# THUDM/GRAND-plus

Measured on AMD Instinct MI355X. Metric: propagation-matrix rows/sec (whole node), higher is better.
Workload: dtype f64

## Files before the change

### grand_plus_amd/csrc/gfpush.hip

```cpp
#include "gfpush_kernels.hpp"
#include "gfpush_sketch.hpp"
#include "gfpush_plan.hpp"
#include "grandplus.h"

#include <dlfcn.h>
#include <sys/prctl.h>
#include <rccl/rccl.h>

#include <algorithm>
#include <atomic>
#include <cmath>
#include <cstdarg>
#include <cstdio>
#include <cstdlib>
#include <cstring>
#include <new>
#include <string>
#include <chrono>
#include <thread>
#include <type_traits>
#include <vector>

using namespace gp;
using namespace gp::planning;
// ... 498 lines not shown
        Held held = g->ws.held();
        bool realloc = false; int need = 0; std::string err;
        Status st;
        while ((st = plan_general(kConsts, in, g->opt, shape, occ, sk, p, g->est, held, &realloc, &need, err)) == kNeedOccupancy) {
            int rc = resident_blocks(general_kernel(p.block_threads), p.block_threads, p.lds_bytes + g->opt.lds_pad, &occ.general[need]);
            if (rc) return rc;
        }
        if (st) return plan_status(st, err);
        if (!realloc) return GP_OK;
        int rc = allocate_workspace(g, held);
        if (rc == GP_ERR_NOMEM && sk.use && !shape.insists_on_sketch()) {
            sk.use = false; g_last_error.clear();
            continue;
        }
        return rc;
    }
}

KParams call_params(const gp_graph* g, const CallArgs& a, const GeneralPlan& gk, u64* counters)
{
    KParams kp;
    std::memset(&kp, 0, sizeof kp);
    kp.indptr = g->d_indptr; kp.indices = g->d_indices; kp.n_nodes = (int)g->n_nodes; kp.nnz = (int)g->nnz;
    kp.deg_shift = g->deg_shift; kp.node_mask = g->node_mask; kp.deg_sat = g->deg_sat;
    kp.seeds = a.d_seeds; kp.n_seeds = a.n_seeds;
    kp.coef = g->d_coef; kp.n_coef = a.n_coef; kp.rmax = a.rmax; kp.K = a.K;
    kp.out_row = a.d_row; kp.out_col = a.d_col; kp.out_val = a.d_val; kp.out_filled = a.d_filled;
    kp.counters = counters;
    kp.lds_slots = gk.lds_slots;
    kp.force_global = g->opt.force_global;
    kp.prune = prune_allowed(g->opt, a.coef, a.n_coef) ? 1 : 0;
    kp.diag_flags = g->opt.diag_flags;
    kp.rows_distinct = g->rows_distinct && g->opt.seedrow ? 1u : 0u;
    kp.solo = (g->opt.solo_levels ? 1u : 0u) | (g->opt.sk_seed_merge ? 2u : 0u);
    kp.direct = direct_tables(g->opt, g->n_nodes, gk) ? 1 : 0;
    return kp;
}

struct GeneralPass { const u32* rows; int n_rows; int queue; u32* overflow; int n_overflow; int overflow_queue; const u32* order; };

int launch_general(const gp_graph* g, KParams& kp, const GeneralPlan& gk, bool gk_acsr, const GeneralPass& pass, hipStream_t s)
{
    const Workspace& w = g->ws;
    const bool two_tier = w.big.n_wg > 0;
    use_csr(kp, g, gk_acsr, true);
    use_slabs(kp, w.est);
    kp.row_map = pass.rows ? pass.rows : pass.order; kp.n_rows_dev = pass.rows ? kp.counters + pass.n_rows : nullptr; kp.queue_counter = pass.queue;
    kp.retry_list = two_tier ? pass.overflow : nullptr; kp.retry_counter = pass.n_overflow;
    const Kernel k = pass.rows ? retry_kernel(gk.block_threads) : general_kernel(gk.block_threads);
    int rc = launch_kernel(k, gk.block_threads, kp, gk.n_wg, gk.lds_bytes + g->opt.lds_pad, s);
    if (rc || !two_tier) return rc;
    use_slabs(kp, w.big);
    kp.row_map = pass.overflow; kp.n_rows_dev = kp.counters + pass.n_overflow; kp.queue_counter = pass.overflow_queue;
    kp.retry_list = nullptr;
    return launch_kernel(retry_kernel(gk.block_threads), gk.block_threads, kp, w.big.n_wg, gk.lds_bytes + g->opt.lds_pad, s);
}

int enqueue_row_order(gp_graph* g, const CallArgs& a, bool acsr, hipStream_t s)
{
    const Workspace& w = g->ws;
    HIP_TRY(hipMemsetAsync(w.order_hist, 0, sizeof(uint32_t) * 64, s));
    const int shift = acsr ? g->a_shift : g->deg_shift;
    const u32 sat = acsr ? g->a_sat : g->deg_sat;
    const unsigned cost_wgs = (unsigned)std::min<int64_t>((a.n_seeds + 15) / 16, 4096), order_wgs = (unsigned)std::min<int64_t>((a.n_seeds + 255) / 256, 1024);
    hipLaunchKernelGGL(row_cost_kernel, dim3(cost_wgs), dim3(256), 0, s, a.d_seeds, (long long)a.n_seeds, (int)g->n_nodes, g->d_indptr,
                       acsr ? g->d_acsr : g->d_indices, acsr ? g->d_node_pos : (const u32*)nullptr, shift, sat, a.rmax, w.cost_cls, w.order_hist);
    hipLaunchKernelGGL(row_order_kernel, dim3(order_wgs), dim3(256), 0, s, w.cost_cls, (long long)a.n_seeds, w.order_hist, w.order_hist + 32, w.order);
// ... 363 lines not shown
            if (!value && g->shared_devices) return fail(GP_ERR_INVALID_ARG, "parts of this handle share a device: RCCL takes one rank per device, the gather stays on the host");
            g->gather_host = value ? 1 : 0; return GP_OK;
        }
        if (k == "min_rows_per_gpu") {
            if (value < 1) return fail(GP_ERR_INVALID_ARG, "min_rows_per_gpu must be >= 1");
            g->min_rows_per_gpu = value; return GP_OK;
        }
        for (gp_graph* q : g->part) if (q) { int rc = gp_set_option(q, key, value); if (rc) return rc; }
        return GP_OK;
    }
    if (k == "block_threads") {
        if (value != 256 && value != 512 && value != 768 && value != 1024) return fail(GP_ERR_INVALID_ARG, "block_threads must be 256, 512, 768 or 1024");
        g->opt.block_threads = (int)value;
    } else if (k == "lds_bytes") {
        if (value < 40 * 1024 || value > 160 * 1024) return fail(GP_ERR_INVALID_ARG, "lds_bytes must be in [40960, 163840]");
        g->opt.lds_bytes = (int)(value & ~15ll);
    } else if (k == "lds_pad") {
        if (value < 0 || value > 120 * 1024) return fail(GP_ERR_INVALID_ARG, "lds_pad must be in [0, 122880]");
        g->opt.lds_pad = (int)(value & ~15ll);
    } else if (k == "kernel") {
        if (value < 0 || value > 2) return fail(GP_ERR_INVALID_ARG, "kernel must be 0 (automatic), 1 (general) or 2 (sketch)");
        g->opt.kernel = (int)value;
    } else if (k == "sk_block_threads") {
        if (value != 0 && value != 512 && value != 768 && value != 1024) return fail(GP_ERR_INVALID_ARG, "sk_block_threads must be 0, 512, 768 or 1024");
        g->opt.sk_block = (int)value;
    } else if (k == "sk_lg_mu" || k == "sk_lg_mr") {
        if (value != 0 && (value < 8 || value > 14)) return fail(GP_ERR_INVALID_ARG, "%s must be 0 or in [8, 14]", key);
        (k == "sk_lg_mu" ? g->opt.sk_lg_mu : g->opt.sk_lg_mr) = (int)value;
    } else if (k == "sk_direct_max") {
        if (value < 0 || value > (1 << 20)) return fail(GP_ERR_INVALID_ARG, "sk_direct_max must be in [0, 2^20]");
        g->opt.sk_direct_max = (int)value;
    } else if (k == "sk_seed_merge") {
        g->opt.sk_seed_merge = value ? 1 : 0;
    } else if (k == "row_order") {
        g->opt.row_order = value ? 1 : 0;
    } else if (k == "gk_acsr") {
        g->opt.gk_acsr = value ? 1 : 0;
    } else if (k == "sk_target") {
        if (value < 0 || value > 4096) return fail(GP_ERR_INVALID_ARG, "sk_target must be in [0, 4096]");
        g->opt.sk_target = (int)value;
    } else if (k == "measure_choice") {
        g->opt.measure_choice = value ? 1 : 0;
        if (!value) g->choices.clear();
    } else if (k == "verify_merge") {
        g->opt.verify_merge = value ? 1 : 0;
    } else if (k == "pretouch") {
        g->opt.pretouch = value ? 1 : 0;
    } else if (k == "max_workgroups") {
        if (value < 0 || value > 65535) return fail(GP_ERR_INVALID_ARG, "max_workgroups must be in [0, 65535]");
        g->opt.max_workgroups = (int)value;
    } else if (k == "workspace_mb") {
        if (value < 1) return fail(GP_ERR_INVALID_ARG, "workspace_mb must be >= 1");
        g->opt.workspace_mb = value;
    } else if (k == "est_level_edges") {
        if (value < 0) return fail(GP_ERR_INVALID_ARG, "est_level_edges must be >= 0");
        g->opt.est_level_edges = value;
    } else if (k == "force_global") {
        g->opt.force_global = value ? 1 : 0;
    } else if (k == "exact_stats") {
        g->opt.exact_stats = value ? 1 : 0;
    } else if (k == "direct_tables") {
        g->opt.direct_tables = value ? 1 : 0;
    } else if (k == "solo_levels") {
        g->opt.solo_levels = value ? 1 : 0;
    } else if (k == "seedrow") {
        g->opt.seedrow = value ? 1 : 0;
// ... 210 lines not shown
    *out = nullptr;
    const int ndev = gp_device_count();
    if (ndev <= 0) return fail(GP_ERR_NO_DEVICE, "no HIP device is visible (this library has no CPU path)");
    if (n_gpus < 0 || n_gpus > ndev) return fail(GP_ERR_NO_DEVICE, "n_gpus = %d but %d device(s) are visible", n_gpus, ndev);
    if (n_gpus == 0) n_gpus = ndev;
    std::vector<int> devs(n_gpus);
    for (int d = 0; d < n_gpus; ++d) devs[d] = d;
    return gp_graph_create_multi_on(indptr, n_nodes, indices, nnz, devs.data(), n_gpus, out);
}

}

namespace {

int replicate_part(gp_graph* g, int d) {
    gp_graph* src = g->part[0];
    HIP_TRY(hipSetDevice(src->device));
    int rc = ensure_packed(src, src->stream);
    if (rc) return rc;
    HIP_TRY(hipStreamSynchronize(src->stream));
    const int dev = g->devices[d];
    HIP_TRY(hipSetDevice(dev));
    hipDeviceProp_t prop;
    HIP_TRY(hipGetDeviceProperties(&prop, dev));
    gp_graph* q = new (std::nothrow) gp_graph();
    if (!q) return fail(GP_ERR_NOMEM, "host allocation failed");
    struct Guard { gp_graph* q; ~Guard() { if (q) gp_graph_destroy(q); } } guard{q};
    q->device = dev; q->n_nodes = src->n_nodes; q->nnz = src->nnz; q->num_cus = prop.multiProcessorCount;
    q->deg_shift = src->deg_shift; q->node_mask = src->node_mask; q->deg_sat = src->deg_sat;
    q->packed = true; q->opt.max_degree_bits = src->opt.max_degree_bits; q->rows_distinct = src->rows_distinct;
    q->opt.block_threads = src->opt.block_threads; q->opt.lds_bytes = src->opt.lds_bytes; q->opt.max_workgroups = src->opt.max_workgroups;
    q->opt.workspace_mb = src->opt.workspace_mb; q->opt.force_global = src->opt.force_global; q->opt.exact_stats = src->opt.exact_stats;
    q->opt.direct_tables = src->opt.direct_tables; q->opt.est_level_edges = src->opt.est_level_edges; q->opt.seedrow = src->opt.seedrow; q->opt.solo_levels = src->opt.solo_levels;
    q->opt.kernel = src->opt.kernel; q->opt.row_order = src->opt.row_order; q->opt.gk_acsr = src->opt.gk_acsr; q->opt.sk_seed_merge = src->opt.sk_seed_merge; q->opt.sk_block = src->opt.sk_block; q->opt.sk_lg_mu = src->opt.sk_lg_mu; q->opt.sk_lg_mr = src->opt.sk_lg_mr; q->opt.sk_target = src->opt.sk_target; q->opt.lds_pad = src->opt.lds_pad; q->opt.sk_direct_max = src->opt.sk_direct_max;
    const size_t b_ptr = sizeof(int) * (size_t)(q->n_nodes + 1), b_idx = sizeof(int) * (size_t)(q->nnz + 1);
    HIP_TRY(hipMalloc(&q->d_indptr, b_ptr));
    HIP_TRY(hipMalloc(&q->d_indices, b_idx));
    if (dev == src->device) {
        HIP_TRY(hipMemcpy(q->d_indptr, src->d_indptr, b_ptr, hipMemcpyDeviceToDevice));
        HIP_TRY(hipMemcpy(q->d_indices, src->d_indices, b_idx, hipMemcpyDeviceToDevice));
    } else {
        HIP_TRY(hipMemcpyPeer(q->d_indptr, dev, src->d_indptr, src->device, b_ptr));
        HIP_TRY(hipMemcpyPeer(q->d_indices, dev, src->d_indices, src->device, b_idx));
    }
    HIP_TRY(hipMalloc(&q->d_counters, sizeof(u64) * kNumCounters));
    HIP_TRY(hipHostMalloc(&q->h_counters, sizeof(u64) * kNumCounters));
    HIP_TRY(hipEventCreate(&q->ev0));
    HIP_TRY(hipEventCreate(&q->ev1));
    HIP_TRY(hipStreamCreateWithFlags(&q->stream, hipStreamNonBlocking));
    guard.q = nullptr;
    g->part[d] = q;
    return GP_OK;
}

int gfpush_multi(gp_graph* g, const int32_t* seeds, int64_t n_seeds, const double* coef, int n_coef, double rmax, int K,
                 int32_t* row_idx, int32_t* col_idx, double* value)
{
    const MultiPlan plan = plan_multi(n_seeds, K, g->n_parts, g->min_rows_per_gpu, g->force_collective != 0, g->gather_host != 0);
    const int G = plan.G, Gc = plan.Gc;
    if (plan.single) {
        int rc = gp_gfpush(g->part[0], seeds, n_seeds, coef, n_coef, rmax, K, row_idx, col_idx, value);
        gp_stats st; const int rc2 = gp_get_stats(g->part[0], &st);
        g->m_last = st; g->m_has_stats = true;
        return rc ? rc : rc2;
    }
    const bool collective = !g->gather_host;
    for (int d = 1; d < Gc; ++d)
// ... 104 lines not shown
```

### grand_plus_amd/csrc/gfpush_plan.hpp

```cpp
#pragma once

#include <algorithm>
#include <atomic>
#include <cmath>
#include <cstddef>
#include <cstdint>
#include <cstdio>
#include <cstring>
#include <string>

namespace gp {
namespace planning {

typedef unsigned long long cap_t;

enum Status { kOk = 0, kInvalidArg, kNoMem, kNeedOccupancy };

struct KernelConsts {
    int ctl_bytes = 0, three_lds = 0, min_cap = 0, topk_bins = 0, bucket_cap = 0, unit_shift = 0;
    int sk_max_pushers = 0, sk_max_coef = 0, sk_tie = 0;
};

struct Options {
    int block_threads = 0; int lds_bytes = 0; int max_workgroups = 0;
    int verify_merge = 0;
    int lds_pad = 0; int pretouch = 0;
    int64_t workspace_mb = 65536; int force_global = 0; int exact_stats = 0; int diag_flags = 0; int direct_tables = 1; int seedrow = 1; int solo_levels = 1;
    int kernel = 0;
    int sk_block = 0, sk_lg_mu = 0, sk_lg_mr = 0, sk_target = 0, sk_direct_max = 0;
    int row_order = 1;
    int sk_seed_merge = 1; int gk_acsr = 1;
    int64_t est_level_edges = 0;
    int measure_choice = 1;
    int max_degree_bits = 31;
};

struct Estimate {
    int kind = 0; int last_kind = 1;
    bool sk_auto_off = false; double sk_off_rmax = 0.0; int sk_off_n_coef = 0;
    bool last_sk_soft = false;
    double edges = 0.0, log = 0.0;
    double rmax = -1.0; int n_coef = 0;
    bool recipe_changed = false;
    double cur_edges = 0.0, cur_log = 0.0;
    int64_t last_call_rows = 0; bool grown_for_call = true;
};


struct SlabCaps {
    int n_wg = 0;
    cap_t push_cap = 0, resg_cap = 0, log_cap = 0, cand_cap = 0, bucket_cap = 0, bt_cap = 0;
    cap_t arch_cap = 0;
    size_t log_bytes() const { return arch_cap ? 6 * (size_t)log_cap + 8 * (size_t)arch_cap : 12 * (size_t)log_cap; }
    size_t per_wg() const { return 16 * (size_t)(2 * push_cap + resg_cap + cand_cap + bucket_cap) + log_bytes() + 8 * (size_t)bt_cap + 64; }
    bool covers(const SlabCaps& o) const {
        if (o.n_wg == 0) return true;
        return n_wg >= o.n_wg && push_cap >= o.push_cap && resg_cap >= o.resg_cap && log_cap >= o.log_cap &&
               cand_cap >= o.cand_cap && bucket_cap >= o.bucket_cap && bt_cap >= o.bt_cap && arch_cap >= o.arch_cap && (arch_cap != 0) == (o.arch_cap != 0);
    }
    void widen(const SlabCaps& o) {
        if (o.n_wg == 0 || (n_wg != 0 && (arch_cap != 0) != (o.arch_cap != 0))) return;
        n_wg = std::max(n_wg, o.n_wg); push_cap = std::max(push_cap, o.push_cap); resg_cap = std::max(resg_cap, o.resg_cap);
        log_cap = std::max(log_cap, o.log_cap); cand_cap = std::max(cand_cap, o.cand_cap); bucket_cap = std::max(bucket_cap, o.bucket_cap);
// ... 422 lines not shown
```

### grand_plus_amd/csrc/gfpush_sketch.hpp

```cpp
#pragma once

#include "gfpush_kernels.hpp"

#ifndef GP_DIAG

namespace gp {

#ifndef GP_SK_SWEEP_DEPTH
#define GP_SK_SWEEP_DEPTH 2
#endif
constexpr int kSkMaxCoef = 40;
constexpr u32 kSkTie     = 256;

struct CtlS {
    long long row;
    LevelCtr lc[2];
    u32 ovf;
    u32 fail;
    u32 n_sel, n_tie;
    u32 tk_bin, tk_above, tk_count, tk_total;
    u32 tk_t, tk_wide, tk_dig;
    u64 kth_bits;
    u32 bcnt[64];
    u64 st[8], st_row[8];
    double coef[kSkMaxCoef + 1];
    u32 cand_q[kSkMaxCoef];
    int seed_key; u32 tot_pu, tot_log;
    double lv_dang; u32 lv_has_dang;
    u32 max_e, max_log;
    u32 k_log_cap, k_pu_cap, k_direct_max, k_solo_ok, k_cx, k_pad; double k_rscale;
#ifdef GP_SK_TIMING
    u64 tacc[16]; u64 tlast;
    u64 tacc2[14]; u64 tlast2;
    u64 t_enter, t_row, row_sum, row_max;
    u64 row_hist[32];
#endif
};
#ifdef GP_SK_TIMING
#define SKT_BEGIN(ctl) do { if (threadIdx.x == 0) (ctl)->tlast = wall_clock64(); } while (0)
#define SKT(ctl, i) do { if (threadIdx.x == 0) { const u64 n_ = wall_clock64(); (ctl)->tacc[i] += n_ - (ctl)->tlast; (ctl)->tlast = n_; } } while (0)
#define SKT_COUNT(ctl, i, n) do { if (threadIdx.x == 0) (ctl)->tacc[i] += (n); } while (0)
#define SKT2_BEGIN(ctl) do { if (threadIdx.x == 0) (ctl)->tlast2 = wall_clock64(); } while (0)
#define SKT2(ctl, i) do { if (threadIdx.x == 0) { const u64 n_ = wall_clock64(); (ctl)->tacc2[i] += n_ - (ctl)->tlast2; (ctl)->tlast2 = n_; } } while (0)
#else
#define SKT_BEGIN(ctl) do { } while (0)
#define SKT(ctl, i) do { } while (0)
#define SKT_COUNT(ctl, i, n) do { } while (0)
#define SKT2_BEGIN(ctl) do { } while (0)
#define SKT2(ctl, i) do { } while (0)
#endif
static_assert(sizeof(CtlS) <= (size_t)kCtlStruct, "the control block must fit its LDS reservation");
enum StatS { zPush = 0, zEdges, zDeg, zFilled, zLevels, zFailed, zCand, zSweep2, zNumStats };
__device__ __forceinline__ void zstat(CtlS* ctl, int which, u64 n) {
    __hip_atomic_fetch_add(&ctl->st_row[which], n, __ATOMIC_RELAXED, __HIP_MEMORY_SCOPE_WORKGROUP);
}

struct SkView {
    CtlS* ctl; u32* R; u32* U; double* xvals; int* xkeys; u32 MU, MR, CX, shU, shR;
    PushEntry* push2; u32* bt2; int* log_key; unsigned short* log_pu; double* arch;
    u32 lds_u;
    u32* bt_l; u32 bt_l_cap;
};
template <int BLOCK>
__device__ __forceinline__ SkView sk_view(KP p, u32 lds0) {
    SkView w;
    w.MU = 1u << p.sk_lg_mu; w.MR = 1u << p.sk_lg_mr; w.CX = p.sk_cx;
    w.shU = 32u - p.sk_lg_mu; w.shR = 32u - p.sk_lg_mr;
    w.ctl = lds_at<CtlS>(lds0);
    w.R = lds_at<u32>(lds0 + (u32)kCtlBytes);
    w.lds_u = lds0 + (u32)kCtlBytes + 4u * w.MR;
    w.U = lds_at<u32>(w.lds_u);
    w.xvals = lds_at<double>(w.lds_u + 4u * w.MU);
    w.xkeys = lds_at<int>(w.lds_u + 4u * w.MU + 8u * w.CX);
    w.bt_l = lds_at<u32>(lds0 + (u32)kCtlStruct + 64u * kFlatW * (u32)(BLOCK / 64));
    w.bt_l_cap = 16u * kFlatW * (16u - (u32)(BLOCK / 64));
    const u32 wg = blockIdx.x;
    w.push2   = p.push + (u64)(2u * wg) * (u32)p.push_cap;
// ... 711 lines not shown
    {
        typedef int    i4 __attribute__((ext_vector_type(4)));
        typedef double d2 __attribute__((ext_vector_type(2)));
        for (u32 base = 0; base < t.CA; base += 4u * BLOCK) {
            const u32 s0 = base + 4u * (u32)tid;
            i4 kk = {kEmpty, kEmpty, kEmpty, kEmpty}; d2 va = {0.0, 0.0}, vb = {0.0, 0.0};
            if (s0 < t.CA) { kk = *(const i4*)&t.akeys[s0]; va = *(const d2*)&t.avals[s0]; vb = *(const d2*)&t.avals[s0 + 2]; }
            const double v[4] = {va.x, va.y, vb.x, vb.y};
#pragma unroll
            for (int j = 0; j < 4; ++j) {
                if (__ballot(kk[j] != kEmpty && v[j] > 0.0) == 0) continue;
                bool is_sel = false, is_t = false;
                Cand cd; cd.bits = (u64)__double_as_longlong(v[j]); cd.key = kk[j]; cd.pad = 0;
                if (kk[j] != kEmpty && v[j] > 0.0) {
                    const u32 id = (u32)cd.key & p.node_mask;
                    const u64 vbits = cd.bits >> vshift;
                    const bool v_eq = vbits == vpre;
                    const bool in_bin = v_eq && (ishift >= 32u || (id >> ishift) == ipre);
                    const bool over = vbits > vpre || (v_eq && ishift < 32u && (id >> ishift) < ipre);
                    is_sel = over || (in_bin && take_all); is_t = in_bin && !take_all;
                }
                const u32 si = wave_alloc1(&ctl->n_sel, is_sel, lane);
                if (is_sel) t.sel[si] = cd;
                const u32 ti = wave_alloc1(&ctl->n_tie, is_t, lane);
                if (is_t) t.tie[ti] = cd;
            }
        }
    }
    GP_SYNC();
    sk_rank_selected<BLOCK>(p, ctl, t, need, take_all, my_rank);
    return need;
}

template <int BLOCK, bool TG>
__device__ GP_PHASE_NOINLINE void phase_sk_topk(u32 lds0, u32 row_lo, u32 row_hi, int seed, u32 n_pu, u32 n_log)
{
    KP p = kparams();
    lds0 = uni(lds0); row_lo = uni(row_lo); row_hi = uni(row_hi); seed = uni(seed); n_pu = uni(n_pu); n_log = uni(n_log);
    const SkView w = sk_view<BLOCK>(p, lds0);
    CtlS* ctl = w.ctl;
    const SkTop t = sk_top(p, w, TG ? 0u : n_pu);
    const long long row = (long long)(((u64)row_hi << 32) | row_lo);
    const int tid = threadIdx.x, lane = tid & 63;
    const u32 wave = wave_id();
    const u32 K = (u32)p.K;

    if (!TG) for (u32 i = tid; i < n_pu; i += BLOCK) t.T[i] = w.arch[i];
    for (u32 i = tid; i < 512u; i += BLOCK) t.fine[i] = 0;
    for (u32 i = tid; i < t.CA; i += BLOCK) { t.akeys[i] = kEmpty; t.avals[i] = 0.0; }
    if (tid < 64) ctl->bcnt[tid] = 0;
    if (tid == 0) { ctl->ovf = 0; ctl->tk_t = 1u; ctl->n_sel = 0; ctl->n_tie = 0; ctl->tk_wide = 0; ctl->kth_bits = ~0ull; }
    bool table_ready = true;
    GP_SYNC();
    for (u32 i = tid; i < t.MR; i += BLOCK) {
        const u32 cv = t.R[i];
        if (cv) {
            const u32 fb = __float_as_uint((float)cv);
            lds_add_u32(&t.fine[min(511u, (fb >> 19) - (127u << 4))], 1u);
        }
    }
    GP_SYNC();
    u32 t_c;
    {
        u32 cnt8[8], sum = 0;
#pragma unroll
        for (int j = 0; j < 8; ++j) { cnt8[j] = t.fine[8 * lane + j]; sum += cnt8[j]; }
        const u32 suf = wave_suffix_scan(sum, lane);
        const u64 m = __ballot(suf >= p.sk_target);
        u32 edge = 1u;
        if (m != 0) {
            const int cl = 63 - __builtin_clzll(m);
            u32 acc = suf - sum; int js = 0;
#pragma unroll
            for (int j = 7; j >= 0; --j) { acc += cnt8[j]; if (acc >= p.sk_target) { js = j; break; } }
            const u32 bin = 8u * (u32)cl + (u32)__builtin_amdgcn_readlane(js, cl), e = bin >> 4, mt = 16u + (bin & 15u);
            edge = max(e >= 4u ? mt << (e - 4u) : mt >> (4u - e), 1u);
        }
        t_c = edge;
    }
    SKT(ctl, 7);
    u32 need = 0, my_rank = 0;
    bool last = false;
    for (int round = 0; ; ++round) {
        u32 P = 1;
        for (;;) {
            bool ovf = false;
            for (u32 part = 0; part < P; ++part) {
                const u32 n_run = part == 0 ? 0u : need;
                Cand mine; mine.bits = 0; mine.key = kEmpty; mine.pad = 0;
                if ((u32)tid < n_run) mine = t.sel[tid];
                if (!table_ready) {
                    GP_SYNC();
                    for (u32 i = tid; i < t.CA; i += BLOCK) { t.akeys[i] = kEmpty; t.avals[i] = 0.0; }
                    if (tid < 64) ctl->bcnt[tid] = 0;
                    if (tid == 0) { ctl->n_sel = 0; ctl->n_tie = 0; ctl->tk_wide = 0; ctl->kth_bits = ~0ull; }
                    GP_SYNC();
                }
                table_ready = false;
                if (n_run != 0u) {
                    if (mine.key != kEmpty) { t.akeys[t.CA - 1u - (u32)tid] = mine.key; t.avals[t.CA - 1u - (u32)tid] = __longlong_as_double((long long)mine.bits); }
                    GP_SYNC();
                }
                auto tabled = [&](const int (&k)[4], const u32 (&pu)[4], auto all_valid) {
                    constexpr bool kAll = decltype(all_valid)::value;
                    u32 cell[4]; double cv[4];
#pragma unroll
                    for (int q = 0; q < 4; ++q) {
                        cell[q] = t.R[sk_cell(kAll ? (u32)k[q] : (u32)max(k[q], 0)) >> t.shR];
                        cv[q] = TG ? w.arch[pu[q]] : t.T[pu[q]];
                    }
                    int kh[4];
#pragma unroll
                    for (int q = 0; q < 4; ++q) kh[q] = (kAll || k[q] >= 0) && cv[q] != 0.0 && cell[q] >= t_c ? k[q] : -1;
                    insert_windows4_asm<true>(t.akeys, t.avals, t.CA, &ctl->ovf, kh, cv, P, part);
                };
#if GP_SK_SWEEP_DEPTH == 2
                log_groups2_nt<BLOCK>(w.log_key, w.log_pu, n_log, tabled);
#else
                log_groups<BLOCK, true>(w.log_key, w.log_pu, 0u, n_log, tabled);
#endif
                GP_SYNC();
                SKT(ctl, 8);
                if (uni(ctl->ovf)) { ovf = true; break; }
                need = sk_select<BLOCK>(p, ctl, t, my_rank);
                SKT(ctl, 9);
                if (need == 0xFFFFFFFFu) { if (tid == 0) ctl->fail = 3; GP_SYNC(); return; }
            }
            if (!ovf) break;
            GP_SYNC();
            if (tid == 0) { ctl->ovf = 0; GP_OVF_COUNT(p, kOvfTopk); }
            P *= 2; need = 0;
            if (P > 64u) { if (tid == 0) ctl->fail = 4; GP_SYNC(); return; }
            GP_SYNC();
        }
        if (t_c <= 1u || last) break;
        if (need == K) {
            const double tau_fx = __builtin_floor(__longlong_as_double((long long)uni(ctl->kth_bits)) * p.sk_rscale * (1.0 - 1.0 / 1048576.0));
            if (tau_fx >= (double)t_c) break;
            t_c = tau_fx >= 1.0 ? (u32)tau_fx : 1u;
            last = true;
        } else {
            t_c = round >= 2 ? 1u : max(1u, t_c >> 4);
        }
        if (tid == 0) zstat(ctl, zSweep2, 1);
    }
    const long long out0 = row * (long long)p.K;
    if ((u32)tid < need) {
        const Cand cd = t.sel[tid];
        const int node = p.unit_info[(u32)cd.key & p.node_mask];
        __builtin_nontemporal_store(seed, &p.out_row[out0 + my_rank]);
        __builtin_nontemporal_store(node, &p.out_col[out0 + my_rank]);
        __builtin_nontemporal_store(__longlong_as_double((long long)cd.bits), &p.out_val[out0 + my_rank]);
    }
    publish_filled(p, row, need);
    if (tid == 0) zstat(ctl, zFilled, need);
}

template <int BLOCK>
__device__ GP_PHASE_NOINLINE void phase_sk_wipe(u32 lds0, u32 what, u32 n, u32 at)
{
    typedef u32 u4 __attribute__((ext_vector_type(4)));
    KP p = kparams();
// ... 187 lines not shown
        if (np == P0 && part == P0) break;
    }
    if (u_dirty) {
        phase_sk_wipe<BLOCK>(lds0, 3u, s_n, cap0);
        GP_SYNC();
    }
    if (uni(ctl->fail)) return 0u;
    if (tid == 0 && !direct) {
        const u32 obs = min(2048u, (u32)(1280.0f * (float)nx->n_rec * __frcp_rn((float)n_rec)) + 8u);
        const u32 old_q = ctl->cand_q[lvl];
        ctl->cand_q[lvl] = max(obs, old_q - (old_q >> 3));
    }
    return 1u;
}

template <int BLOCK>
__device__ GP_PHASE_NOINLINE u32 phase_sk_level1_redo(u32 lds0, u32 L) { return phase_sk_level<BLOCK, true>(lds0, 1u, L); }

template <int BLOCK>
__device__ __forceinline__ void gfpush_sk_rows()
{
    extern __shared__ __attribute__((aligned(16))) unsigned char smem[];
    KP p = kparams();
    const u32 lds0 = uni(lds_addr(smem));
    const SkView w = sk_view<BLOCK>(p, lds0);
    CtlS* ctl = w.ctl;
    const int tid = threadIdx.x;
    phase_sk_wipe<BLOCK>(lds0, 1u, 0u, 0u);
    if (tid < 8) { ctl->st[tid] = 0; ctl->st_row[tid] = 0; }
#ifdef GP_SK_TIMING
    if (tid < 16) ctl->tacc[tid] = 0;
    if (tid < 14) ctl->tacc2[tid] = 0;
    if (tid < 32) ctl->row_hist[tid] = 0;
    if (tid == 0) { ctl->t_enter = wall_clock64(); ctl->row_sum = 0; ctl->row_max = 0; }
#endif
    if (tid < kSkMaxCoef) { ctl->cand_q[tid] = 0; if (tid < p.n_coef) ctl->coef[tid] = p.coef[tid]; }
    if (tid == 0) {
        ctl->max_e = 0; ctl->max_log = 0;
        ctl->k_log_cap = (u32)min(p.log_cap, (u64)0xFFFFFFFFu); ctl->k_pu_cap = (u32)min((u64)kSkMaxPushers, p.arch_cap);
        ctl->k_direct_max = min(p.sk_direct_max, 3u * (w.CX / 4u)); ctl->k_cx = w.CX; ctl->k_rscale = p.sk_rscale;
        ctl->k_solo_ok = (p.solo & 1u) && p.push_cap >= (u64)kSkSoloEdges + 4u &&
                         (double)p.bt_cap >= (p.rmax > 0.0 ? fmin((double)p.nnz, 1.001 / p.rmax + 16.0) : (double)p.nnz) / (double)(1u << kUnitShift) + 4.0 ? 1u : 0u;
    }
    const long long n_rows = p.n_seeds;
    const u32 L = (u32)p.n_coef - 1u;

    for (;;) {
        GP_SYNC();
        SKT_BEGIN(ctl);
        if (tid == 0) {
            long long q = (long long)__hip_atomic_fetch_add(&p.counters[p.queue_counter], 1ull, __ATOMIC_RELAXED, __HIP_MEMORY_SCOPE_AGENT);
            if (p.row_map && q < n_rows) q = (long long)p.row_map[q];
            ctl->row = q;
            ctl->fail = 0; ctl->ovf = 0;
#ifdef GP_SK_TIMING
            ctl->t_row = ctl->tlast;
#endif
        }
        GP_SYNC();
        const long long row = uni(ctl->row);
        if (row >= n_rows) break;
        const int seed = uni(p.seeds[row]);
        if (seed < 0 || seed >= p.n_nodes) {
            if (tid == 0) { __hip_atomic_fetch_add(&ctl->st[zFailed], 1ull, __ATOMIC_RELAXED, __HIP_MEMORY_SCOPE_WORKGROUP); if (p.out_filled) p.out_filled[row] = 0; }
            continue;
        }
        u32 lvl = 1u + uni(phase_sk_seed<BLOCK>(lds0, seed));
        GP_SYNC();
        SKT(ctl, 0); SKT_COUNT(ctl, 15, 1);
        if (lvl == 2u) {
            SKT_COUNT(ctl, 13, 1);
            if (uni(ctl->ovf)) lvl = uni(phase_sk_level1_redo<BLOCK>(lds0, L)) ? 2u : L + 1u;
        }
        for (; lvl <= L; ++lvl)
            if (!uni(phase_sk_level<BLOCK>(lds0, lvl, L))) break;
        GP_SYNC();
        SKT(ctl, 6);
        if (!uni(ctl->fail)) {
            const u32 n_pu = uni(ctl->tot_pu), n_log = uni(ctl->tot_log);
            if (tid == 0) ctl->max_log = max(ctl->max_log, n_log);
            const u32 top_region = 4u * w.MU + 12u * w.CX;
            if (2u * sk_top_slots(top_region, n_pu, (u32)p.K) >= sk_top_slots(top_region, 0u, (u32)p.K))
                 phase_sk_topk<BLOCK, false>(lds0, (u32)(u64)row, (u32)((u64)row >> 32), seed, n_pu, n_log);
            else phase_sk_topk<BLOCK, true>(lds0, (u32)(u64)row, (u32)((u64)row >> 32), seed, n_pu, n_log);
        }
        GP_SYNC();
        if (uni(ctl->fail)) {
            if (tid == 0) {
                const u64 i = __hip_atomic_fetch_add(&p.counters[p.retry_counter], 1ull, __ATOMIC_RELAXED, __HIP_MEMORY_SCOPE_AGENT);
                p.retry_list[i] = (u32)row;
                if (ctl->fail == 1) __hip_atomic_fetch_add(&p.counters[kSkSlabFails], 1ull, __ATOMIC_RELAXED, __HIP_MEMORY_SCOPE_AGENT);
#ifndef GP_SK_TIMING
                __hip_atomic_fetch_add(&p.counters[kDiag0 + min(ctl->fail, 7u)], 1ull, __ATOMIC_RELAXED, __HIP_MEMORY_SCOPE_AGENT);
#endif
            }
            if (tid < 8) ctl->st_row[tid] = 0;
        } else if (tid < 8) { ctl->st[tid] += ctl->st_row[tid]; ctl->st_row[tid] = 0; }
        GP_SYNC();
        phase_sk_wipe<BLOCK>(lds0, 1u, 0u, 0u);
        SKT(ctl, 10);
#ifdef GP_SK_TIMING
        if (tid == 0) {
            const u64 dt = ctl->tlast - ctl->t_row;
            ctl->row_sum += dt; ctl->row_max = max(ctl->row_max, dt); ++ctl->row_hist[min(31u, 63u - (u32)__builtin_clzll(dt | 1ull))];
        }
#endif
    }
#ifdef GP_SK_TIMING
    if (tid == 0 && p.wg_log) { p.wg_log[2u * blockIdx.x] = ctl->t_enter; p.wg_log[2u * blockIdx.x + 1u] = wall_clock64(); }
#endif
    GP_SYNC();
    if (tid == 0) {
        const Counter dst[zNumStats] = { kPushes, kEdges, kDegLookups, kFilled, kLdsLevels, kFailedRows, kSkCandEdges, kSkSweep2 };
#pragma unroll
        for (int i = 0; i < zNumStats; ++i)
            if (ctl->st[i]) __hip_atomic_fetch_add(&p.counters[dst[i]], ctl->st[i], __ATOMIC_RELAXED, __HIP_MEMORY_SCOPE_AGENT);
        if (ctl->max_e) __hip_atomic_fetch_max(&p.counters[kMaxLevelEdges], (u64)ctl->max_e, __ATOMIC_RELAXED, __HIP_MEMORY_SCOPE_AGENT);
        if (ctl->max_log) __hip_atomic_fetch_max(&p.counters[kMaxLogRecords], (u64)ctl->max_log, __ATOMIC_RELAXED, __HIP_MEMORY_SCOPE_AGENT);
#ifdef GP_SK_TIMING
        for (int i = 0; i < 16; ++i) __hip_atomic_fetch_add(&p.counters[kDiag0 + i], ctl->tacc[i], __ATOMIC_RELAXED, __HIP_MEMORY_SCOPE_AGENT);
        for (int i = 0; i < 14; ++i) __hip_atomic_fetch_add(&p.counters[kDiagX0 + i], ctl->tacc2[i], __ATOMIC_RELAXED, __HIP_MEMORY_SCOPE_AGENT);
        __hip_atomic_fetch_add(&p.counters[kDiagX0 + 16], ctl->row_sum, __ATOMIC_RELAXED, __HIP_MEMORY_SCOPE_AGENT);
        __hip_atomic_fetch_max(&p.counters[kDiagX0 + 17], ctl->row_max, __ATOMIC_RELAXED, __HIP_MEMORY_SCOPE_AGENT);
        for (int i = 0; i < 32; ++i)
            if (ctl->row_hist[i]) __hip_atomic_fetch_add(&p.counters[kDiagX0 + 32 + i], ctl->row_hist[i], __ATOMIC_RELAXED, __HIP_MEMORY_SCOPE_AGENT);
#endif
    }
}

template <int BLOCK>
__global__ void __launch_bounds__(BLOCK, BLOCK == 1024 ? 4 : 6) gfpush_sk_kernel(const KParams)
{
    gfpush_sk_rows<BLOCK>();
}

}

#endif
```

Measured before the change: 3.586 million.

## Add hash-bucketed top-k partitioning after first overflow in sketch kernel

When the single-pass top-k selection overflows its LDS window, the new default path estimates the number of distinct candidate keys with a bitmap cardinality sketch. It then scatters the log records into hash buckets in place and runs selection bucket by bucket, merging survivors. This replaces repeated full-log sweeps with doubling partition counts. It adds two extra log passes plus bitmap work per overflowing row and makes the kernel's control flow more complex.

```diff
diff --git a/grand_plus_amd/csrc/gfpush.hip b/grand_plus_amd/csrc/gfpush.hip
--- a/grand_plus_amd/csrc/gfpush.hip
+++ b/grand_plus_amd/csrc/gfpush.hip
@@ -554,7 +554,8 @@
     kp.prune = prune_allowed(g->opt, a.coef, a.n_coef) ? 1 : 0;
     kp.diag_flags = g->opt.diag_flags;
     kp.rows_distinct = g->rows_distinct && g->opt.seedrow ? 1u : 0u;
-    kp.solo = (g->opt.solo_levels ? 1u : 0u) | (g->opt.sk_seed_merge ? 2u : 0u);
+    kp.solo = (g->opt.solo_levels ? 1u : 0u) | (g->opt.sk_seed_merge ? 2u : 0u) |
+              (g->opt.sk_topk_buckets ? 4u : 0u) | (g->opt.sk_topk_buckets == 2 ? 8u : 0u);
     kp.direct = direct_tables(g->opt, g->n_nodes, gk) ? 1 : 0;
     return kp;
 }
@@ -984,6 +985,9 @@
         g->opt.sk_direct_max = (int)value;
     } else if (k == "sk_seed_merge") {
         g->opt.sk_seed_merge = value ? 1 : 0;
+    } else if (k == "sk_topk_buckets") {
+        if (value < 0 || value > 2) return fail(GP_ERR_INVALID_ARG, "sk_topk_buckets must be 0, 1 or 2");
+        g->opt.sk_topk_buckets = (int)value;
     } else if (k == "row_order") {
         g->opt.row_order = value ? 1 : 0;
     } else if (k == "gk_acsr") {
@@ -1260,7 +1264,7 @@
     q->opt.block_threads = src->opt.block_threads; q->opt.lds_bytes = src->opt.lds_bytes; q->opt.max_workgroups = src->opt.max_workgroups;
     q->opt.workspace_mb = src->opt.workspace_mb; q->opt.force_global = src->opt.force_global; q->opt.exact_stats = src->opt.exact_stats;
     q->opt.direct_tables = src->opt.direct_tables; q->opt.est_level_edges = src->opt.est_level_edges; q->opt.seedrow = src->opt.seedrow; q->opt.solo_levels = src->opt.solo_levels;
-    q->opt.kernel = src->opt.kernel; q->opt.row_order = src->opt.row_order; q->opt.gk_acsr = src->opt.gk_acsr; q->opt.sk_seed_merge = src->opt.sk_seed_merge; q->opt.sk_block = src->opt.sk_block; q->opt.sk_lg_mu = src->opt.sk_lg_mu; q->opt.sk_lg_mr = src->opt.sk_lg_mr; q->opt.sk_target = src->opt.sk_target; q->opt.lds_pad = src->opt.lds_pad; q->opt.sk_direct_max = src->opt.sk_direct_max;
+    q->opt.kernel = src->opt.kernel; q->opt.row_order = src->opt.row_order; q->opt.gk_acsr = src->opt.gk_acsr; q->opt.sk_seed_merge = src->opt.sk_seed_merge; q->opt.sk_topk_buckets = src->opt.sk_topk_buckets; q->opt.sk_block = src->opt.sk_block; q->opt.sk_lg_mu = src->opt.sk_lg_mu; q->opt.sk_lg_mr = src->opt.sk_lg_mr; q->opt.sk_target = src->opt.sk_target; q->opt.lds_pad = src->opt.lds_pad; q->opt.sk_direct_max = src->opt.sk_direct_max;
     const size_t b_ptr = sizeof(int) * (size_t)(q->n_nodes + 1), b_idx = sizeof(int) * (size_t)(q->nnz + 1);
     HIP_TRY(hipMalloc(&q->d_indptr, b_ptr));
     HIP_TRY(hipMalloc(&q->d_indices, b_idx));
diff --git a/grand_plus_amd/csrc/gfpush_plan.hpp b/grand_plus_amd/csrc/gfpush_plan.hpp
--- a/grand_plus_amd/csrc/gfpush_plan.hpp
+++ b/grand_plus_amd/csrc/gfpush_plan.hpp
@@ -29,6 +29,7 @@
     int kernel = 0;
     int sk_block = 0, sk_lg_mu = 0, sk_lg_mr = 0, sk_target = 0, sk_direct_max = 0;
     int row_order = 1;
+    int sk_topk_buckets = 1;
     int sk_seed_merge = 1; int gk_acsr = 1;
     int64_t est_level_edges = 0;
     int measure_choice = 1;
diff --git a/grand_plus_amd/csrc/gfpush_sketch.hpp b/grand_plus_amd/csrc/gfpush_sketch.hpp
--- a/grand_plus_amd/csrc/gfpush_sketch.hpp
+++ b/grand_plus_amd/csrc/gfpush_sketch.hpp
@@ -34,6 +34,8 @@
     u64 tacc2[14]; u64 tlast2;
     u64 t_enter, t_row, row_sum, row_max;
     u64 row_hist[32];
+    u64 sw_rows[8], sw_ticks[8];
+    u32 tk_sweeps, tk_pad;
 #endif
 };
 #ifdef GP_SK_TIMING
@@ -42,7 +44,9 @@
 #define SKT_COUNT(ctl, i, n) do { if (threadIdx.x == 0) (ctl)->tacc[i] += (n); } while (0)
 #define SKT2_BEGIN(ctl) do { if (threadIdx.x == 0) (ctl)->tlast2 = wall_clock64(); } while (0)
 #define SKT2(ctl, i) do { if (threadIdx.x == 0) { const u64 n_ = wall_clock64(); (ctl)->tacc2[i] += n_ - (ctl)->tlast2; (ctl)->tlast2 = n_; } } while (0)
+#define SKT_SWEEP(ctl) do { if (threadIdx.x == 0) ++(ctl)->tk_sweeps; } while (0)
 #else
+#define SKT_SWEEP(ctl) do { } while (0)
 #define SKT_BEGIN(ctl) do { } while (0)
 #define SKT(ctl, i) do { } while (0)
 #define SKT_COUNT(ctl, i, n) do { } while (0)
@@ -820,7 +824,142 @@
     return need;
 }
 
+constexpr u32 kSkBktRank = 800u;
 template <int BLOCK, bool TG>
+__device__ GP_PHASE_NOINLINE void phase_sk_topk_buckets(u32 lds0, u32 n_pu, u32 n_log)
+{
+    KP p = kparams();
+    lds0 = uni(lds0); n_pu = uni(n_pu); n_log = uni(n_log);
+    const SkView w = sk_view<BLOCK>(p, lds0);
+    CtlS* ctl = w.ctl;
+    const SkTop t = sk_top(p, w, TG ? 0u : n_pu);
+    const int tid = threadIdx.x, lane = tid & 63;
+    u32* cnt = t.fine + 512u; u32* pre = t.fine + 576u; u32* cur = t.fine + 648u; u32* lim = t.fine + 712u; u32* hdr = t.fine + 776u;
+    const u32 t_c = uni(ctl->tk_t);
+    u32* bm = (u32*)t.avals;
+    const u32 bm_words = 1u << (31u - (u32)__builtin_clz(2u * t.CA));
+    for (u32 i = tid; i < bm_words; i += BLOCK) bm[i] = 0;
+    if (tid < 64) cnt[tid] = 0;
+    if (tid == 0) { hdr[0] = 0; hdr[1] = 0; hdr[2] = 0; ctl->tk_above = 0; }
+    GP_SYNC();
+    auto passes = [&](const int (&k)[4], const u32 (&pu)[4], bool (&ok)[4]) {
+        u32 cell[4]; double cv[4];
+#pragma unroll
+        for (int q = 0; q < 4; ++q) {
+            cell[q] = t.R[sk_cell((u32)max(k[q], 0)) >> t.shR];
+            cv[q] = TG ? w.arch[pu[q]] : t.T[pu[q]];
+        }
+#pragma unroll
+        for (int q = 0; q < 4; ++q) ok[q] = k[q] >= 0 && cv[q] != 0.0 && cell[q] >= t_c;
+    };
+    log_groups<BLOCK, false>(w.log_key, w.log_pu, 0u, n_log, [&](const int (&k)[4], const u32 (&pu)[4], auto) {
+        bool ok[4];
+        passes(k, pu, ok);
+#pragma unroll
+        for (int q = 0; q < 4; ++q) if (ok[q]) {
+            const u32 h = hash_b((u32)k[q]);
+            lds_add_u32(&cnt[h >> 26], 1u);
+            __hip_atomic_fetch_or(&bm[(h >> 5) & (bm_words - 1u)], 1u << (h & 31u), __ATOMIC_RELAXED, __HIP_MEMORY_SCOPE_WORKGROUP);
+        }
+    });
+    GP_SYNC();
+    {
+        u32 ones = 0;
+        for (u32 i = tid; i < bm_words; i += BLOCK) ones += (u32)__popc(bm[i]);
+        ones = wave_sum32(ones);
+        if (lane == 0 && ones) lds_add_u32(&hdr[2], ones);
+    }
+    GP_SYNC();
+    SKT(ctl, 8); SKT_SWEEP(ctl);
+    if (tid < 64) {
+        const u32 incl = wave_incl_scan_dpp(cnt[lane]);
+        if (lane == 0) { pre[0] = 0; ctl->tk_total = 0; }
+        pre[lane + 1] = incl;
+        __atomic_signal_fence(__ATOMIC_SEQ_CST);
+        const u32 total = (u32)__builtin_amdgcn_readlane((int)incl, 63);
+        const float m_bits = 32.0f * (float)bm_words, clear = m_bits - (float)hdr[2];
+        const float est = clear >= 1.0f ? -m_bits * __logf(clear / m_bits) * 1.03f + 32.0f : (float)total;
+        const u32 nodes = min(total, (u32)est);
+        const u32 fit = 9u * (t.CA / 16u);
+        u32 lgP = 1;
+        while (lgP <= 6u && nodes > (fit << lgP)) ++lgP;
+        if (lgP <= 6u) {
+            const u32 g = 64u >> lgP;
+            const u32 c = (u32)lane < (1u << lgP) ? pre[((u32)lane + 1u) * g] - pre[(u32)lane * g] : 0u;
+            const u32 c4 = (c + 3u) & ~3u;
+            const u32 incl4 = wave_incl_scan_dpp(c4);
+            const u64 first = (((u64)n_log + 3u) & ~3ull) + (incl4 - c4);
+            const u64 end_all = (((u64)n_log + 3u) & ~3ull) + (u32)__builtin_amdgcn_readlane((int)incl4, 63);
+            const bool room = end_all <= (u64)ctl->k_log_cap && (p.solo & 8u) == 0u;
+            if (room) {
+                if ((u32)lane < (1u << lgP)) { cur[lane] = (u32)first; lim[lane] = (u32)first + c; }
+                if (lane == 0) hdr[0] = lgP;
+            }
+        }
+    }
+    GP_SYNC();
+    const u32 lgP = uni(hdr[0]);
+    if (lgP == 0u) return;
+    const u32 P = 1u << lgP;
+    log_groups<BLOCK, true>(w.log_key, w.log_pu, 0u, n_log, [&](const int (&k)[4], const u32 (&pu)[4], auto) {
+        bool ok[4];
+        passes(k, pu, ok);
+#pragma unroll
+        for (int q = 0; q < 4; ++q) if (ok[q]) {
+            const u32 b = hash_b((u32)k[q]) >> (32u - lgP);
+            const u32 at = __hip_atomic_fetch_add(&cur[b], 1u, __ATOMIC_RELAXED, __HIP_MEMORY_SCOPE_WORKGROUP);
+            if (at < lim[b]) { w.log_key[at] = k[q]; w.log_pu[at] = (unsigned short)pu[q]; }
+            else hdr[1] = 1u;
+        }
+    });
+    GP_SYNC();
+    SKT(ctl, 8); SKT_SWEEP(ctl);
+    if (uni(hdr[1])) return;
+    u32 need = 0, my_rank = 0;
+    for (u32 part = 0; part < P; ++part) {
+        const u32 n_run = part == 0 ? 0u : need;
+        Cand mine; mine.bits = 0; mine.key = kEmpty; mine.pad = 0;
+        if ((u32)tid < n_run) mine = t.sel[tid];
+        GP_SYNC();
+        for (u32 i = tid; i < t.CA; i += BLOCK) { t.akeys[i] = kEmpty; t.avals[i] = 0.0; }
+        if (tid < 64) ctl->bcnt[tid] = 0;
+        if (tid == 0) { ctl->n_sel = 0; ctl->n_tie = 0; ctl->tk_wide = 0; ctl->kth_bits = ~0ull; }
+        GP_SYNC();
+        if (n_run != 0u) {
+            if (mine.key != kEmpty) { t.akeys[t.CA - 1u - (u32)tid] = mine.key; t.avals[t.CA - 1u - (u32)tid] = __longlong_as_double((long long)mine.bits); }
+            GP_SYNC();
+        }
+        const u32 b_end = uni(lim[part]), b_first = b_end - (uni(pre[(part + 1u) * (64u >> lgP)]) - uni(pre[part * (64u >> lgP)]));
+        if (b_end > b_first)
+            log_groups<BLOCK, true>(w.log_key, w.log_pu, b_first, b_end, [&](const int (&k)[4], const u32 (&pu)[4], auto) {
+                double cv[4];
+#pragma unroll
+                for (int q = 0; q < 4; ++q) cv[q] = TG ? w.arch[pu[q]] : t.T[pu[q]];
+                insert_windows4_asm<true>(t.akeys, t.avals, t.CA, &ctl->ovf, k, cv, 1u, 0u);
+            });
+        GP_SYNC();
+        SKT(ctl, 8);
+        if (uni(ctl->ovf)) {
+            GP_SYNC();
+            if (tid == 0) ctl->ovf = 0;
+            GP_SYNC();
+            return;
+        }
+        need = sk_select<BLOCK>(p, ctl, t, my_rank);
+        SKT(ctl, 9);
+        if (need == 0xFFFFFFFFu) { if (tid == 0) ctl->fail = 3; GP_SYNC(); return; }
+    }
+    if ((u32)tid < need) t.fine[kSkBktRank + (u32)tid] = my_rank;
+    if (tid == 0) {
+        ctl->tk_above = 1u; ctl->tk_count = need;
+#ifndef GP_SK_TIMING
+        __hip_atomic_fetch_add(&p.counters[kDiag0 + 11], 1ull, __ATOMIC_RELAXED, __HIP_MEMORY_SCOPE_AGENT);
+#endif
+    }
+    GP_SYNC();
+}
+
+template <int BLOCK, bool TG, bool REST = false>
 __device__ GP_PHASE_NOINLINE void phase_sk_topk(u32 lds0, u32 row_lo, u32 row_hi, int seed, u32 n_pu, u32 n_log)
 {
     KP p = kparams();
@@ -833,12 +972,19 @@
     const u32 wave = wave_id();
     const u32 K = (u32)p.K;
 
+    u32 t_c, need, my_rank, P0 = 1u;
+    bool last = false, table_ready = true, skip = false;
+    int round = 0;
+    if (REST) {
+        t_c = uni(ctl->tk_t); round = (int)uni(ctl->tk_dig); last = uni(ctl->tk_bin) != 0u; table_ready = false; need = 0; my_rank = 0;
+        if (uni(ctl->tk_above)) { skip = true; need = uni(ctl->tk_count); if ((u32)tid < need) my_rank = t.fine[kSkBktRank + (u32)tid]; }
+        else { P0 = 2u; if (tid == 0) GP_OVF_COUNT(p, kOvfTopk); }
+    } else {
     if (!TG) for (u32 i = tid; i < n_pu; i += BLOCK) t.T[i] = w.arch[i];
     for (u32 i = tid; i < 512u; i += BLOCK) t.fine[i] = 0;
     for (u32 i = tid; i < t.CA; i += BLOCK) { t.akeys[i] = kEmpty; t.avals[i] = 0.0; }
     if (tid < 64) ctl->bcnt[tid] = 0;
-    if (tid == 0) { ctl->ovf = 0; ctl->tk_t = 1u; ctl->n_sel = 0; ctl->n_tie = 0; ctl->tk_wide = 0; ctl->kth_bits = ~0ull; }
-    bool table_ready = true;
+    if (tid == 0) { ctl->ovf = 0; ctl->tk_t = 1u; ctl->tk_total = 0; ctl->n_sel = 0; ctl->n_tie = 0; ctl->tk_wide = 0; ctl->kth_bits = ~0ull; }
     GP_SYNC();
     for (u32 i = tid; i < t.MR; i += BLOCK) {
         const u32 cv = t.R[i];
@@ -848,7 +994,6 @@
         }
     }
     GP_SYNC();
-    u32 t_c;
     {
         u32 cnt8[8], sum = 0;
 #pragma unroll
@@ -867,12 +1012,13 @@
         t_c = edge;
     }
     SKT(ctl, 7);
-    u32 need = 0, my_rank = 0;
-    bool last = false;
-    for (int round = 0; ; ++round) {
-        u32 P = 1;
+    need = 0; my_rank = 0;
+    }
+    for (;; ++round) {
+        u32 P = P0; P0 = 1u;
         for (;;) {
             bool ovf = false;
+            if (!skip)
             for (u32 part = 0; part < P; ++part) {
                 const u32 n_run = part == 0 ? 0u : need;
                 Cand mine; mine.bits = 0; mine.key = kEmpty; mine.pad = 0;
@@ -908,14 +1054,20 @@
                 log_groups<BLOCK, true>(w.log_key, w.log_pu, 0u, n_log, tabled);
 #endif
                 GP_SYNC();
-                SKT(ctl, 8);
+                SKT(ctl, 8); SKT_SWEEP(ctl);
                 if (uni(ctl->ovf)) { ovf = true; break; }
                 need = sk_select<BLOCK>(p, ctl, t, my_rank);
                 SKT(ctl, 9);
                 if (need == 0xFFFFFFFFu) { if (tid == 0) ctl->fail = 3; GP_SYNC(); return; }
             }
+            skip = false;
             if (!ovf) break;
             GP_SYNC();
+            if (P == 1u && (p.solo & 4u)) {
+                if (tid == 0) { ctl->ovf = 0; ctl->tk_t = t_c; ctl->tk_dig = (u32)round; ctl->tk_bin = last ? 1u : 0u; ctl->tk_total = 1u; }
+                GP_SYNC();
+                return;
+            }
             if (tid == 0) { ctl->ovf = 0; GP_OVF_COUNT(p, kOvfTopk); }
             P *= 2; need = 0;
             if (P > 64u) { if (tid == 0) ctl->fail = 4; GP_SYNC(); return; }
@@ -1169,6 +1321,7 @@
     if (tid < 16) ctl->tacc[tid] = 0;
     if (tid < 14) ctl->tacc2[tid] = 0;
     if (tid < 32) ctl->row_hist[tid] = 0;
+    if (tid < 8) { ctl->sw_rows[tid] = 0; ctl->sw_ticks[tid] = 0; }
     if (tid == 0) { ctl->t_enter = wall_clock64(); ctl->row_sum = 0; ctl->row_max = 0; }
 #endif
     if (tid < kSkMaxCoef) { ctl->cand_q[tid] = 0; if (tid < p.n_coef) ctl->coef[tid] = p.coef[tid]; }
@@ -1191,7 +1344,7 @@
             ctl->row = q;
             ctl->fail = 0; ctl->ovf = 0;
 #ifdef GP_SK_TIMING
-            ctl->t_row = ctl->tlast;
+            ctl->t_row = ctl->tlast; ctl->tk_sweeps = 0;
 #endif
         }
         GP_SYNC();
@@ -1217,11 +1370,16 @@
             const u32 n_pu = uni(ctl->tot_pu), n_log = uni(ctl->tot_log);
             if (tid == 0) ctl->max_log = max(ctl->max_log, n_log);
             const u32 top_region = 4u * w.MU + 12u * w.CX;
-            if (2u * sk_top_slots(top_region, n_pu, (u32)p.K) >= sk_top_slots(top_region, 0u, (u32)p.K))
-                 phase_sk_topk<BLOCK, false>(lds0, (u32)(u64)row, (u32)((u64)row >> 32), seed, n_pu, n_log);
-            else phase_sk_topk<BLOCK, true>(lds0, (u32)(u64)row, (u32)((u64)row >> 32), seed, n_pu, n_log);
-        }
-        GP_SYNC();
+            const bool t_fits = 2u * sk_top_slots(top_region, n_pu, (u32)p.K) >= sk_top_slots(top_region, 0u, (u32)p.K);
+            if (t_fits) phase_sk_topk<BLOCK, false>(lds0, (u32)(u64)row, (u32)((u64)row >> 32), seed, n_pu, n_log);
+            else        phase_sk_topk<BLOCK, true>(lds0, (u32)(u64)row, (u32)((u64)row >> 32), seed, n_pu, n_log);
+            GP_SYNC();
+            while (uni(ctl->tk_total) && !uni(ctl->fail)) {
+                if (t_fits) { phase_sk_topk_buckets<BLOCK, false>(lds0, n_pu, n_log); phase_sk_topk<BLOCK, false, true>(lds0, (u32)(u64)row, (u32)((u64)row >> 32), seed, n_pu, n_log); }
+                else        { phase_sk_topk_buckets<BLOCK, true>(lds0, n_pu, n_log);  phase_sk_topk<BLOCK, true, true>(lds0, (u32)(u64)row, (u32)((u64)row >> 32), seed, n_pu, n_log); }
+                GP_SYNC();
+            }
+        } else GP_SYNC();
         if (uni(ctl->fail)) {
             if (tid == 0) {
                 const u64 i = __hip_atomic_fetch_add(&p.counters[p.retry_counter], 1ull, __ATOMIC_RELAXED, __HIP_MEMORY_SCOPE_AGENT);
@@ -1240,6 +1398,8 @@
         if (tid == 0) {
             const u64 dt = ctl->tlast - ctl->t_row;
             ctl->row_sum += dt; ctl->row_max = max(ctl->row_max, dt); ++ctl->row_hist[min(31u, 63u - (u32)__builtin_clzll(dt | 1ull))];
+            const u32 ns = ctl->tk_sweeps, sb = ns <= 2u ? ns : min(6u, 33u - (u32)__builtin_clz(ns - 1u));
+            ++ctl->sw_rows[sb]; ctl->sw_ticks[sb] += dt;
         }
 #endif
     }
@@ -1261,6 +1421,11 @@
         __hip_atomic_fetch_max(&p.counters[kDiagX0 + 17], ctl->row_max, __ATOMIC_RELAXED, __HIP_MEMORY_SCOPE_AGENT);
         for (int i = 0; i < 32; ++i)
             if (ctl->row_hist[i]) __hip_atomic_fetch_add(&p.counters[kDiagX0 + 32 + i], ctl->row_hist[i], __ATOMIC_RELAXED, __HIP_MEMORY_SCOPE_AGENT);
+        for (int i = 0; i < 7; ++i)
+            if (ctl->sw_rows[i]) {
+                __hip_atomic_fetch_add(&p.counters[kDiagX0 + 64 + i], ctl->sw_rows[i], __ATOMIC_RELAXED, __HIP_MEMORY_SCOPE_AGENT);
+                __hip_atomic_fetch_add(&p.counters[kDiagX0 + 72 + i], ctl->sw_ticks[i], __ATOMIC_RELAXED, __HIP_MEMORY_SCOPE_AGENT);
+            }
 #endif
     }
 }
```

New measurement: 3.605 million (median of 6 runs). About the same (+0.5%).
